# joomanzi/cleisthenes

Hardware: AMD Instinct MI355X
Metric: RBC shard GB/s (RS encode+decode + Merkle verify) per GPU & node, N=128 (higher is better)
Workload: dtype u8

## Files before the change

cleisthenes_amd/csrc/capi.cpp:

```cpp
#include <dlfcn.h>
#include <hip/hip_runtime_api.h>
#include <limits.h>
#include <rccl/rccl.h>
#include <stdio.h>
#include <string.h>

#include <stdlib.h>

#include <algorithm>
#include <functional>
#include <memory>
#include <mutex>
#include <thread>
#include <unordered_map>
#include <vector>

#include "../../include/rbc_gpu.h"
#include "../../include/rbc_protocol.h"
#include "gf_host.h"
#include "kernels.h"
#include "wire_session.h"

namespace {

constexpr size_t kAlign = 64;
inline size_t round_up(size_t x, size_t a) { return (x + a - 1) / a * a; }

int tree_width(int n) {
    int w = 1;
    while (w < n) w <<= 1;
    return w;
}
int tree_depth(int n) {
    int w = tree_width(n), d = 0;
    while ((1 << d) < w) ++d;
    return d;
}

#define RBC_HIP(expr)                                  \
    do {                                               \
        hipError_t e_ = (expr);                        \
        if (e_ != hipSuccess) return RBC_ERR_DEVICE;   \
    } while (0)

struct DevBuf {
    void *p = nullptr;
    size_t cap = 0;
    bool pinned = false;
    hipError_t ensure(size_t bytes) {
        if (bytes <= cap && p) return hipSuccess;
        release();
        size_t want = std::max(bytes, (size_t)256);
        hipError_t e = pinned ? hipHostMalloc(&p, want, hipHostMallocDefault) : hipMalloc(&p, want);
        if (e != hipSuccess) { p = nullptr; cap = 0; return e; }
        cap = want;
        return hipSuccess;
    }
    void release() {
        if (p) {
            if (pinned) (void)hipHostFree(p);
            else (void)hipFree(p);
        }
        p = nullptr;
        cap = 0;
    }
    template <class T> T *as() const { return reinterpret_cast<T *>(p); }
};

struct Ws {
    DevBuf used, regen, dmat, nmiss, flags, list, counter, rcount, cls, vleaves, vlist;
    DevBuf vroot[2], need_full;
    DevBuf rxcnt;
    int rx_par = 0;
    bool rxcnt_init = false, v_clean[2] = {true, true};
    int rx_vslot = 0;
    bool rx_vreuse = false;
    bool fork = true;
    int rx_count = 0;
    const uint8_t *rx_shards = nullptr;
    hipStream_t aux = nullptr;
    hipEvent_t ev_fork = nullptr, ev_join = nullptr, ev_hashed = nullptr, ev_rel = nullptr;
    bool init() {
        return hipEventCreateWithFlags(&ev_fork, hipEventDisableTiming) == hipSuccess &&
               hipEventCreateWithFlags(&ev_join, hipEventDisableTiming) == hipSuccess &&
               hipEventCreateWithFlags(&ev_hashed, hipEventDisableTiming) == hipSuccess &&
               hipEventCreateWithFlags(&ev_rel, hipEventDisableTiming) == hipSuccess;
    }
    void release() {
        for (DevBuf *b : {&used, &regen, &dmat, &nmiss, &flags, &list, &counter, &rcount, &cls, &vleaves, &vlist,
                          &vroot[0], &vroot[1], &need_full, &rxcnt})
            b->release();
        if (aux) (void)hipStreamDestroy(aux);
        if (ev_fork) (void)hipEventDestroy(ev_fork);
        if (ev_join) (void)hipEventDestroy(ev_join);
        if (ev_hashed) (void)hipEventDestroy(ev_hashed);
        if (ev_rel) (void)hipEventDestroy(ev_rel);
        aux = nullptr;
        ev_fork = ev_join = ev_hashed = ev_rel = nullptr;
    }
};

struct Slot {
    DevBuf d_values, d_shards, d_leaves, d_roots, d_branches, d_valid, d_status, d_digests, d_lens, d_slens, d_idx,
        d_offs, d_present, d_pack, d_parity;
    DevBuf h_in{nullptr, 0, true}, h_out{nullptr, 0, true};
    Ws ws;
    hipStream_t stream = nullptr;
    hipEvent_t done = nullptr;
    hipEvent_t kdone = nullptr;
    uint64_t ticket = 0;
    bool busy = false;
    std::function<int()> finish;
    std::function<int(hipStream_t)> d2h;
    int d2h_rc = 0;
    void release() {
        for (DevBuf *b : {&d_values, &d_shards, &d_leaves, &d_roots, &d_branches, &d_valid, &d_status, &d_digests,
                          &d_lens, &d_slens, &d_idx, &d_offs, &d_present, &d_pack, &d_parity, &h_in, &h_out})
            b->release();
        ws.release();
        if (stream) (void)hipStreamDestroy(stream);
        if (done) (void)hipEventDestroy(done);
        if (kdone) (void)hipEventDestroy(kdone);
        stream = nullptr;
        done = nullptr;
        kdone = nullptr;
    }
};

#ifndef RBC_HOST_SLOTS
#define RBC_HOST_SLOTS 4
#endif
constexpr int kHostSlots = RBC_HOST_SLOTS;

}

struct rbc_ctx {
    int n = 0, f = 0, k = 0, p = 0, depth = 0, width = 0, device = 0;
    bool fft = false;
    bool fft_generic = false;
    bool fft_wide = false;
    bool fft_small = false;
    int fft_lane = 0;
    int tx_prio = 0, rx_prio = 0;
    int gemv_prio_ = -1, reencode_prio_ = -1;
    int recheck = RBC_RECHECK_REUSE;
    int wire_codec = RBC_WIRE_CODEC_JSON;
    int gemv_prio() const { return gemv_prio_ < 0 ? tx_prio : gemv_prio_; }
    int reencode_prio() const { return reencode_prio_ < 0 ? tx_prio : reencode_prio_; }
    std::vector<uint8_t> h_M;
    uint8_t *d_M = nullptr;
    std::mutex mu;
    hipStream_t stream = nullptr;
    Ws ws;
    DevBuf d_values, d_shards, d_valid, d_status;
    DevBuf h_stage{nullptr, 0, true};
    uint64_t next_ticket = 1;
    std::vector<std::unique_ptr<Slot>> slots;
    std::unordered_map<uint64_t, int> retired;
    ncclComm_t comm = nullptr;
    int nranks = 1, rank = 0;
    DevBuf d_pack;
};

struct rbc_rs {
    rbc_ctx *ctx = nullptr;
};

namespace {

int ctx_create_kn(int n, int k, int device, rbc_ctx **out) {
    if (!out) return RBC_ERR_INVALID_ARG;
    *out = nullptr;
    if (k <= 0 || n - k < 0) return RBC_ERR_INV_SHARD_NUM;
    if (n > 256) return RBC_ERR_MAX_SHARD_NUM;
    int ndev = 0;
    if (hipGetDeviceCount(&ndev) != hipSuccess || device < 0 || device >= ndev) return RBC_ERR_DEVICE;
    rbc_ctx *c = new rbc_ctx();
    c->n = n;
    c->k = k;
    c->p = n - k;
    c->f = (n - k) / 2;
// ... 183 lines not shown
    return stage_merkle_build(c, st, count, leaves, roots, branches);
}

static bool shared_path_verify(const rbc_ctx *c, const uint32_t *shard_lens, uint32_t uniform_shard_len) {
    const uint32_t blocks_per_row = shard_lens ? 0u : (uniform_shard_len + 9 + 63) / 64;
    return (shard_lens || 16u * (uint32_t)c->depth >= blocks_per_row) && c->depth >= 1;
}

void *ws_buffer(rbc_ctx *c, Ws *wsp, DevBuf Ws::*buf, size_t bytes) {
    std::unique_lock<std::mutex> lk(c->mu, std::defer_lock);
    if (!wsp) lk.lock();
    Ws &w = wsp ? *wsp : c->ws;
    DevBuf &b = w.*buf;
    return b.ensure(bytes) == hipSuccess ? b.p : nullptr;
}

struct EchoVerify {
    uint32_t *counter = nullptr;
    bool zero_counter = true;
    uint8_t *roots_keep = nullptr;
    ShaArgs sha{};
    bool path = false;

    int plan(rbc_ctx *c, hipStream_t st, int count, const Rows &b, const uint8_t *branches, const uint8_t *roots,
             const uint8_t *present, uint8_t *valid, uint8_t *leaves, Ws *wsp) {
        sha = sha_args(c, count, b, leaves, c->rx_prio);
        sha.rows_per_inst = c->n;
        sha.branches = branches;
        sha.br_inst_pitch = (uint64_t)c->n * c->depth * 32;
        sha.roots = roots;
        sha.present = present;
        sha.valid = valid;
        if (present) {
            uint32_t *vl = (uint32_t *)ws_buffer(c, wsp, &Ws::vlist, (size_t)count * c->n * 4 + 64);
            if (!vl) return RBC_ERR_DEVICE;
            uint32_t *vc = counter ? counter : vl + (size_t)count * c->n;
            if (zero_counter) RBC_HIP(hipMemsetAsync(vc, 0, 4, st));
            RBC_HIP(rbc_launch_compact_present(present, c->n, count, valid, vl, vc, st, c->rx_prio,
                                               roots_keep ? roots : nullptr, roots_keep));
            sha.list = vl;
            sha.list_count = vc;
        }
        path = shared_path_verify(c, b.lens, b.uniform_len);
        if (path && !leaves) {
            sha.leaves = (uint8_t *)ws_buffer(c, wsp, &Ws::vleaves, (size_t)count * c->n * 32);
            if (!sha.leaves) return RBC_ERR_DEVICE;
        }
        return RBC_OK;
    }
    int finish(const rbc_ctx *c, hipStream_t st) const {
        if (!path) return RBC_OK;
        PathArgs p{};
        p.count = sha.count;
        p.n = c->n;
        p.width = c->width;
        p.lg_width = c->depth;
        p.depth = c->depth;
        p.leaves = sha.leaves;
        p.leaves_inst_pitch = sha.leaves_inst_pitch;
        p.branches = sha.branches;
        p.br_inst_pitch = sha.br_inst_pitch;
        p.roots = sha.roots;
        p.present = sha.present;
        p.valid = sha.valid;
        p.prio = sha.prio;
        RBC_HIP(rbc_launch_merkle_path(p, st));
        return RBC_OK;
    }
};

int stage_verify(rbc_ctx *c, hipStream_t st, int count, const Rows &b, const uint8_t *branches, const uint8_t *roots,
                 const uint8_t *present, uint8_t *valid, uint8_t *leaves, Ws *wsp = nullptr) {
    if (count < 0 || (count > 0 && (!b.rows || !roots || !valid || (c->depth > 0 && !branches))))
        return RBC_ERR_INVALID_ARG;
    if (!b.rows_ok()) return RBC_ERR_INVALID_ARG;
    if (count == 0) return RBC_OK;
    EchoVerify ev;
    int rc = ev.plan(c, st, count, b, branches, roots, present, valid, leaves, wsp);
    if (rc) return rc;
    RBC_HIP(rbc_launch_sha_rows(ev.sha, !ev.path, st));
    return ev.finish(c, st);
}

int ensure_ws(rbc_ctx *c, Ws &w, int count) {
    const size_t nr = (size_t)std::max(c->n - c->k, 1);
    RBC_HIP(w.used.ensure((size_t)count * c->k));
    RBC_HIP(w.regen.ensure((size_t)count * nr));
    RBC_HIP(w.dmat.ensure((size_t)count * nr * c->k));
    RBC_HIP(w.nmiss.ensure((size_t)count * 4));
    RBC_HIP(w.flags.ensure((size_t)count * c->n * 4));
    RBC_HIP(w.list.ensure((size_t)count * nr * 4));
    RBC_HIP(w.counter.ensure(16));
    RBC_HIP(w.rcount.ensure((size_t)count * 4));
    RBC_HIP(w.cls.ensure((size_t)count * round_up(c->n, 4)));
    return RBC_OK;
}

GfArgs decode_gf_args(const rbc_ctx *c, int count, const Rows &b, const PrepArgs &pa) {
    GfArgs g{};
    g.count = count;
    g.K = c->k;
    g.mode = GF_MODE_DECODE;
    g.in = b.rows;
    g.in_inst_pitch = b.inst_pitch(c);
    g.in_row_pitch = b.pitch;
    g.in_inst_bytes = (uint32_t)b.inst_pitch(c);
    g.out = b.rows;
    g.out_inst_pitch = b.inst_pitch(c);
    g.out_row_pitch = b.pitch;
    g.lens = b.lens;
    g.uniform_len = b.uniform_len;
    g.coef = pa.dmat;
    g.coef_inst_stride = pa.dmat_stride;
    g.in_idx = pa.used;
    g.out_idx = pa.regen;
    g.idx_stride = pa.used_stride;
    g.idx_stride2 = pa.regen_stride;
    g.status = pa.status;
    return g;
}

constexpr uint32_t kFusedJoinMinS = 2048;
int stage_regenerate(rbc_ctx *c, Ws &w, hipStream_t st, int count, const Rows &b, const uint8_t *valid,
                     int32_t *status, int compare = 0, uint32_t *zeroed_counter = nullptr,
                     uint8_t *values_out = nullptr, uint32_t value_pitch = 0, bool *joined = nullptr) {
    if (joined) *joined = false;
    int rc = ensure_ws(c, w, count);
    if (rc) return rc;
    uint32_t *counter = zeroed_counter ? zeroed_counter : w.counter.as<uint32_t>();
    if (compare && !zeroed_counter) RBC_HIP(hipMemsetAsync(counter, 0, 16, st));
    const int nr = c->n - c->k;
    PrepArgs pa{};
    pa.count = count;
    pa.n = c->n;
    pa.k = c->k;
    pa.valid = valid;
    pa.valid_stride = (uint32_t)c->n;
    pa.M = c->d_M;
    pa.used = w.used.as<uint8_t>();
    pa.used_stride = (uint32_t)c->k;
    pa.regen = w.regen.as<uint8_t>();
    pa.regen_stride = (uint32_t)std::max(nr, 1);
    pa.dmat = w.dmat.as<uint8_t>();
    pa.dmat_stride = (uint64_t)std::max(nr, 1) * c->k;
    pa.status = status;
    pa.prio = c->rx_prio;
    if (compare) {
        pa.nmiss = w.nmiss.as<int32_t>();
        pa.flags = w.flags.as<uint32_t>();
        pa.list = w.list.as<uint32_t>();
        pa.counter = counter;
    }
    if (c->fft) {
        pa.fft = 1;
        pa.rcount = w.rcount.as<int32_t>();
        pa.cls = w.cls.as<uint8_t>();
        pa.cls_stride = (uint32_t)round_up(c->n, 4);
        pa.gf_exp = c->d_M + c->h_M.size();
        pa.gf_log = pa.gf_exp + 512;
    }
    RBC_HIP(rbc_launch_decode_prepare(pa, st));
    if (c->fft && nr > 0) {
        const int rmax = std::min(c->k, nr);
        GfArgs g = decode_gf_args(c, count, b, pa);
        g.R = rmax;
        g.rcount = pa.rcount;
        g.prio = c->gemv_prio();
        RBC_HIP(rbc_launch_gf_regen(g, st));
        FftArgs a{};
        a.count = count;
        a.n = c->n;
        a.k = c->k;
        a.mode = GF_MODE_DECODE;
        a.shards = b.rows;
        a.inst_pitch = b.inst_pitch(c);
        a.row_pitch = b.pitch;
        a.lens = b.lens;
        a.uniform_len = b.uniform_len;
        a.status = status;
        a.cls = pa.cls;
        a.cls_stride = pa.cls_stride;
        if (compare) {
            a.flags = pa.flags;
            a.list = pa.list;
            a.counter = pa.counter;
        }
        a.prio = c->reencode_prio();
        a.generic = c->fft_generic;
        a.lane = c->fft_lane;
        if (values_out && joined && !c->fft_generic && !b.lens && b.uniform_len >= kFusedJoinMinS &&
            value_pitch >= (uint64_t)c->k * b.uniform_len &&
            value_pitch - (uint64_t)c->k * b.uniform_len <= std::min<uint64_t>(256, b.pitch)) {
            a.join = values_out;
            a.join_pitch = value_pitch;
            *joined = true;
        }
        RBC_HIP(rbc_launch_rs_fft(a, st));
    } else if (nr > 0) {
        GfArgs g = decode_gf_args(c, count, b, pa);
        g.tiles = (int)((b.pitch + 4095) / 4096);
        g.R = nr;
        g.rc = rbc_gf_pick_rc(nr, kGfRcMax);
        if (compare) {
            g.nmiss = pa.nmiss;
            g.flags = pa.flags;
            g.list = pa.list;
            g.counter = pa.counter;
            g.n = c->n;
        }
        g.prio = c->reencode_prio();
        RBC_HIP(rbc_launch_gf_rows(g, st));
    }
    return RBC_OK;
}

struct JoinBack {
    Ws &w;
    hipStream_t st;
    bool armed = false;
    bool record = true;
    ~JoinBack() {
        if (!armed) return;
        if (record) (void)hipEventRecord(w.ev_join, w.aux);
        (void)hipStreamWaitEvent(st, w.ev_join, 0);
    }
};

int launch_join(rbc_ctx *c, hipStream_t js, int count, const Rows &b, uint8_t *values_out, uint32_t value_pitch,
                const int32_t *status) {
    JoinArgs j{};
    j.count = count;
    j.k = c->k;
// ... 56 lines not shown
        ds = w.aux;
    }
    RBC_HIP(rbc_launch_merkle(m, true, st));
    if (digests)
        RBC_HIP(rbc_launch_digest(leaves, (uint64_t)c->n * 32, c->k, status, digests, count, ds, c->rx_prio));
    return RBC_OK;
}

Rows rx_rows(const rbc_rx_batch *b) { return {b->shards, b->shard_pitch, b->shard_lens, b->uniform_shard_len}; }

int check_rx_batch(rbc_ctx *c, const rbc_rx_batch *b) {
    if (b->count < 0) return RBC_ERR_INVALID_ARG;
    if (b->count == 0) return RBC_OK;
    if (!b->shards || !b->roots || !b->valid || !b->leaves || !b->status || (c->depth > 0 && !b->branches))
        return RBC_ERR_INVALID_ARG;
    return rx_rows(b).decode_ok(c, b->values_out, b->value_pitch) ? RBC_OK : RBC_ERR_INVALID_ARG;
}

bool rx_alias(const rbc_rx_batch *a, const rbc_rx_batch *b) {
    auto same = [](const void *x, const void *y) { return x && x == y; };
    return same(a->shards, b->shards) || same(a->leaves, b->leaves) || same(a->status, b->status) ||
           same(a->valid, b->valid) || same(a->values_out, b->values_out) || same(a->digests, b->digests);
}

int stage_receive_step(rbc_ctx *c, hipStream_t st, const rbc_rx_batch *cur, const rbc_rx_batch *prev,
                       const rbc_rx_marks *marks) {
    Ws &w = c->ws;
    int rc;
    if (cur && (rc = check_rx_batch(c, cur))) return rc;
    if (prev && (rc = check_rx_batch(c, prev))) return rc;
    const bool hc = cur && cur->count > 0, hp = prev && prev->count > 0;
    if (hp != (w.rx_count > 0) || (hp && (prev->count != w.rx_count || prev->shards != w.rx_shards)))
        return RBC_ERR_INVALID_ARG;
    if (hc && hp && rx_alias(cur, prev)) return RBC_ERR_INVALID_ARG;
    if (!hc && !hp) return RBC_OK;
    if (!aux_stream(w)) return RBC_ERR_DEVICE;
    const int nr = c->n - c->k;
    EchoVerify ev;
    ShaArgs r{};
    ev.sha.prio = c->rx_prio;
    RBC_HIP(w.rxcnt.ensure(64));
    if (!w.rxcnt_init) {
        RBC_HIP(hipMemsetAsync(w.rxcnt.p, 0, 64, st));
        w.rxcnt_init = true;
        w.v_clean[0] = w.v_clean[1] = true;
    }
    const int par = w.rx_par;
    uint32_t *cnt = w.rxcnt.as<uint32_t>();
    uint32_t *v_cnt = cnt + 4 * par, *v_next = cnt + 4 * (par ^ 1), *r_cnt = cnt + 8 + 4 * par,
             *r_prev = cnt + 8 + 4 * (par ^ 1);
    const bool reuse = c->recheck == RBC_RECHECK_REUSE && c->depth >= 1;
    const int cur_vslot = w.rx_vslot ^ (hp ? 1 : 0);
    bool roots_kept = false;
    if (hc && reuse) RBC_HIP(w.vroot[cur_vslot].ensure((size_t)cur->count * 32));
    const bool hv = hc && !cur->verified;
    if (hv) {
        ev.counter = v_cnt;
        ev.zero_counter = !w.v_clean[par];
        ev.roots_keep = reuse ? w.vroot[cur_vslot].as<uint8_t>() : nullptr;
        rc = ev.plan(c, st, cur->count, rx_rows(cur), cur->branches, cur->roots, cur->present, cur->valid, cur->leaves,
                     &w);
        if (rc) return rc;
        if (cur->present) {
            w.v_clean[par] = false;
            roots_kept = reuse;
        }
    }
    if (hp && nr > 0) {
        r = sha_args(c, prev->count, rx_rows(prev), prev->leaves, c->rx_prio);
        r.rows_per_inst = nr;
        r.status = prev->status;
        r.list = w.list.as<uint32_t>();
        r.list_count = r_prev;
    }
    if (hc && reuse && !roots_kept)
        RBC_HIP(hipMemcpyAsync(w.vroot[cur_vslot].p, cur->roots, (size_t)cur->count * 32, hipMemcpyDeviceToDevice, st));
    if (marks && marks->hash_begin) RBC_HIP(hipEventRecord((hipEvent_t)marks->hash_begin, st));
    RBC_HIP(rbc_launch_sha_rx(ev.sha, r, hv && !ev.path, st, reinterpret_cast<uint4 *>(r_cnt),
                              reinterpret_cast<uint4 *>(v_next)));
    w.v_clean[par ^ 1] = true;
    if (marks && marks->rows_hashed) RBC_HIP(hipEventRecord((hipEvent_t)marks->rows_hashed, st));
    if ((rc = ev.finish(c, st))) return rc;
    if (marks && marks->hashed) RBC_HIP(hipEventRecord((hipEvent_t)marks->hashed, st));
    JoinBack pj{w, st, false, false};
    if (hp) {
        if (prev->digests) {
            RBC_HIP(hipEventRecord(w.ev_hashed, st));
            RBC_HIP(hipStreamWaitEvent(w.aux, w.ev_hashed, 0));
            RBC_HIP(rbc_launch_digest(prev->leaves, (uint64_t)c->n * 32, c->k, prev->status, prev->digests,
                                      prev->count, w.aux, c->rx_prio));
        }
        RBC_HIP(hipEventRecord(w.ev_join, w.aux));
        pj.armed = true;
        MerkleArgs m = merkle_check_args(c, prev->count, prev->leaves, prev->roots, prev->status);
        if (reuse && w.rx_vreuse) {
            RBC_HIP(w.need_full.ensure((size_t)prev->count));
            RecheckArgs ra{};
            ra.count = prev->count;
            ra.n = c->n;
            ra.width = c->width;
            ra.depth = c->depth;
            ra.leaves = prev->leaves;
            ra.leaves_inst_pitch = (uint64_t)c->n * 32;
            ra.branches = prev->branches;
            ra.br_inst_pitch = (uint64_t)c->n * c->depth * 32;
            ra.valid = prev->valid;
            ra.flags = w.flags.as<uint32_t>();
            ra.vroots = w.vroot[w.rx_vslot].as<uint8_t>();
            ra.expect_roots = prev->roots;
            ra.status = prev->status;
            ra.need_full = w.need_full.as<uint8_t>();
            ra.prio = c->rx_prio;
            RBC_HIP(rbc_launch_recheck(ra, st));
            m.only = ra.need_full;
        }
        RBC_HIP(rbc_launch_merkle(m, true, st));
        if (marks && marks->prev_released) {
            RBC_HIP(hipEventRecord(w.ev_rel, st));
            RBC_HIP(hipStreamWaitEvent(w.aux, w.ev_rel, 0));
            RBC_HIP(hipEventRecord((hipEvent_t)marks->prev_released, w.aux));
        }
    }
    w.rx_count = 0;
    if (hc) {
        if (marks && marks->decode_begin) RBC_HIP(hipEventRecord((hipEvent_t)marks->decode_begin, st));
        bool joined = false;
        rc = stage_regenerate(c, w, st, cur->count, rx_rows(cur), cur->valid, cur->status, 1, r_cnt, cur->values_out,
                              cur->value_pitch, &joined);
        if (rc) return rc;
        if (marks && marks->decoded) RBC_HIP(hipEventRecord((hipEvent_t)marks->decoded, st));
        if (cur->values_out && !joined) {
            RBC_HIP(hipEventRecord(w.ev_fork, st));
            RBC_HIP(hipStreamWaitEvent(w.aux, w.ev_fork, 0));
            rc = launch_join(c, w.aux, cur->count, rx_rows(cur), cur->values_out, cur->value_pitch, cur->status);
            if (rc) return rc;
        }
        w.rx_count = cur->count;
        w.rx_shards = cur->shards;
        w.rx_vslot = cur_vslot;
        w.rx_vreuse = reuse;
    }
    w.rx_par ^= 1;
    return RBC_OK;
}

int check_shards(const size_t *lens, int n, bool nilok, size_t *size_out) {
    size_t size = 0;
    for (int i = 0; i < n; ++i)
        if (lens[i]) { size = lens[i]; break; }
    if (size == 0) return RBC_ERR_SHARD_NO_DATA;
    for (int i = 0; i < n; ++i)
        if (lens[i] != size && (lens[i] != 0 || !nilok)) return RBC_ERR_SHARD_SIZE;
    *size_out = size;
    return RBC_OK;
}

int host_reconstruct(rbc_ctx *c, uint8_t *const *shards, size_t *lens, int n_shards, bool data_only) {
    if (!shards || !lens) return RBC_ERR_INVALID_ARG;
    if (n_shards != c->n) return RBC_ERR_TOO_FEW_SHARDS;
    size_t S = 0;
    int rc = check_shards(lens, n_shards, true, &S);
    if (rc) return rc;
    int present = 0;
    for (int i = 0; i < c->n; ++i) {
        if (lens[i] && !shards[i]) return RBC_ERR_INVALID_ARG;
        present += lens[i] != 0;
    }
    if (present == c->n) return RBC_OK;
    if (present < c->k) return RBC_ERR_TOO_FEW_SHARDS;
    if (S > 0x7fffffffULL / (size_t)c->n) return RBC_ERR_INVALID_ARG;
    const size_t pitch = round_up(S, kAlign);
    std::lock_guard<std::mutex> lk(c->mu);
    RBC_HIP(hipSetDevice(c->device));
    RBC_HIP(c->d_shards.ensure((size_t)c->n * pitch));
    RBC_HIP(c->d_valid.ensure((size_t)c->n));
    RBC_HIP(c->d_status.ensure(sizeof(int32_t)));
    RBC_HIP(c->h_stage.ensure((size_t)c->n * pitch + c->n));
    uint8_t *stage = c->h_stage.as<uint8_t>();
    memset(stage, 0, (size_t)c->n * pitch + c->n);
    for (int i = 0; i < c->n; ++i) {
        if (lens[i]) memcpy(stage + (size_t)i * pitch, shards[i], S);
        stage[(size_t)c->n * pitch + i] = lens[i] ? 1 : 0;
    }
    hipStream_t st = host_stream(c);
    if (!st) return RBC_ERR_DEVICE;
    RBC_HIP(hipMemcpyAsync(c->d_shards.p, stage, (size_t)c->n * pitch, hipMemcpyHostToDevice, st));
    RBC_HIP(hipMemcpyAsync(c->d_valid.p, stage + (size_t)c->n * pitch, c->n, hipMemcpyHostToDevice, st));
    rc = stage_regenerate(c, c->ws, st, 1, {c->d_shards.as<uint8_t>(), (uint32_t)pitch, nullptr, (uint32_t)S},
                          c->d_valid.as<uint8_t>(), c->d_status.as<int32_t>());
    if (rc) return rc;
    RBC_HIP(hipMemcpyAsync(stage, c->d_shards.p, (size_t)c->n * pitch, hipMemcpyDeviceToHost, st));
    int32_t status = 0;
    RBC_HIP(hipMemcpyAsync(&status, c->d_status.p, sizeof status, hipMemcpyDeviceToHost, st));
    RBC_HIP(hipStreamSynchronize(st));
    if (status) return status;
    const int last = data_only ? c->k : c->n;
    for (int i = 0; i < last; ++i) {
        if (lens[i]) continue;
        if (!shards[i]) return RBC_ERR_INVALID_ARG;
        memcpy(shards[i], stage + (size_t)i * pitch, S);
        lens[i] = S;
    }
    return RBC_OK;
}

}

extern "C" {

const char *rbc_strerror(int s) {
    switch (s) {
// ... 1731 lines not shown
```

cleisthenes_amd/csrc/device_common.h:

```cpp
#pragma once
#include <hip/hip_runtime.h>
#include <stdint.h>

#define RBC_DEV __device__ __forceinline__

RBC_DEV void set_wave_prio(int p) {
    if (p == 1) __builtin_amdgcn_s_setprio(1);
    else if (p == 2) __builtin_amdgcn_s_setprio(2);
    else if (p >= 3) __builtin_amdgcn_s_setprio(3);
}

namespace rbcdev {

RBC_DEV uint32_t rotr(uint32_t x, uint32_t n) { return __builtin_amdgcn_alignbit(x, x, n); }
RBC_DEV uint32_t xor3(uint32_t a, uint32_t b, uint32_t c) {
    return __builtin_amdgcn_bitop3_b32(a, b, c, 0x96);
}
RBC_DEV uint32_t bswap32(uint32_t x) { return __builtin_amdgcn_perm(0u, x, 0x00010203u); }
RBC_DEV uint32_t perm(uint32_t hi, uint32_t lo, uint32_t sel) { return __builtin_amdgcn_perm(hi, lo, sel); }

__constant__ static const uint32_t kSHA_K[64] = {
    0x428a2f98, 0x71374491, 0xb5c0fbcf, 0xe9b5dba5, 0x3956c25b, 0x59f111f1, 0x923f82a4, 0xab1c5ed5,
    0xd807aa98, 0x12835b01, 0x243185be, 0x550c7dc3, 0x72be5d74, 0x80deb1fe, 0x9bdc06a7, 0xc19bf174,
    0xe49b69c1, 0xefbe4786, 0x0fc19dc6, 0x240ca1cc, 0x2de92c6f, 0x4a7484aa, 0x5cb0a9dc, 0x76f988da,
// ... 230 lines not shown
#pragma unroll
    for (int r = 0; r < 2; ++r)
#pragma unroll
        for (int t = 0; t < 8; ++t) out[r][t] = s[r].h[t];
}

RBC_DEV void sha256_node64(const uint32_t (&l)[8], const uint32_t (&r)[8], uint32_t (&out)[8]) {
    Sha256State s;
    sha256_init(s);
    uint32_t w[16];
#pragma unroll
    for (int t = 0; t < 8; ++t) { w[t] = l[t]; w[8 + t] = r[t]; }
    sha256_compress(s, w);
#pragma unroll
    for (int t = 0; t < 16; ++t) w[t] = 0;
    w[0] = 0x80000000u;
    w[15] = 512u;
    sha256_compress(s, w);
#pragma unroll
    for (int t = 0; t < 8; ++t) out[t] = s.h[t];
}

RBC_DEV void sha256_node32(const uint32_t (&l)[8], uint32_t (&out)[8]) {
    Sha256State s;
    sha256_init(s);
    uint32_t w[16];
#pragma unroll
    for (int t = 0; t < 8; ++t) w[t] = l[t];
    w[8] = 0x80000000u;
#pragma unroll
    for (int t = 9; t < 15; ++t) w[t] = 0;
    w[15] = 256u;
    sha256_compress(s, w);
#pragma unroll
    for (int t = 0; t < 8; ++t) out[t] = s.h[t];
}

RBC_DEV void sha256_empty(uint32_t (&out)[8]) {
    out[0] = 0xe3b0c442u; out[1] = 0x98fc1c14u; out[2] = 0x9afbf4c8u; out[3] = 0x996fb924u;
    out[4] = 0x27ae41e4u; out[5] = 0x649b934cu; out[6] = 0xa495991bu; out[7] = 0x7852b855u;
}

RBC_DEV void store_digest(uint8_t *dst, const uint32_t (&h)[8]) {
    uint4 *q = reinterpret_cast<uint4 *>(dst);
    q[0] = make_uint4(bswap32(h[0]), bswap32(h[1]), bswap32(h[2]), bswap32(h[3]));
    q[1] = make_uint4(bswap32(h[4]), bswap32(h[5]), bswap32(h[6]), bswap32(h[7]));
}
RBC_DEV void load_digest(const uint8_t *src, uint32_t (&h)[8]) {
    const uint4 *q = reinterpret_cast<const uint4 *>(src);
    const uint4 a = q[0], b = q[1];
    h[0] = bswap32(a.x); h[1] = bswap32(a.y); h[2] = bswap32(a.z); h[3] = bswap32(a.w);
    h[4] = bswap32(b.x); h[5] = bswap32(b.y); h[6] = bswap32(b.z); h[7] = bswap32(b.w);
}

RBC_DEV uint32_t gf_xtime(uint32_t v) { return ((v << 1) ^ ((v & 0x80u) ? 0x1du : 0u)) & 0xffu; }

RBC_DEV void gf_tables(uint32_t c, uint4 &t01, uint32_t &t2) {
    uint32_t m[8];
    m[0] = c & 0xffu;
#pragma unroll
    for (int i = 1; i < 8; ++i) m[i] = gf_xtime(m[i - 1]);
    const uint32_t t0lo = (m[0] << 8) | (m[1] << 16) | ((m[0] ^ m[1]) << 24);
    const uint32_t t0hi = m[2] | ((m[2] ^ m[0]) << 8) | ((m[2] ^ m[1]) << 16) | ((m[2] ^ m[1] ^ m[0]) << 24);
    const uint32_t t1lo = (m[3] << 8) | (m[4] << 16) | ((m[3] ^ m[4]) << 24);
    const uint32_t t1hi = m[5] | ((m[5] ^ m[3]) << 8) | ((m[5] ^ m[4]) << 16) | ((m[5] ^ m[4] ^ m[3]) << 24);
    t01 = make_uint4(t0lo, t0hi, t1lo, t1hi);
    t2 = (m[6] << 8) | (m[7] << 16) | ((m[6] ^ m[7]) << 24);
}

struct GfSel {
    uint32_t s0, s1, s2;
};
RBC_DEV GfSel gf_sel(uint32_t x) {
    GfSel s;
    s.s0 = x & 0x07070707u;
    s.s1 = (x >> 3) & 0x07070707u;
    s.s2 = (x >> 6) & 0x03030303u;
    return s;
}
RBC_DEV uint32_t gf_mul4(const uint4 &t01, uint32_t t2, const GfSel &s) {
    return xor3(perm(t01.y, t01.x, s.s0), perm(t01.w, t01.z, s.s1), perm(t2, t2, s.s2));
}

}
```

cleisthenes_amd/csrc/gf_regen.hip:

```cpp
#include <algorithm>

#include "buffer_io.h"
#include "kernels.h"

using namespace rbcdev;

template <int W>
struct GfVec {
    uint32_t v[W];
};
template <int I, int MAX, class F>
__device__ __forceinline__ void dispatch_rows(int rows, F &&f) {
    if constexpr (I <= MAX) {
        if (rows == I) f(IntC<I>{});
        else dispatch_rows<I + 1, MAX>(rows, f);
    }
}

template <int W, int RC, int JC, int NT, int WPE>
__global__ __launch_bounds__(64 * NT) __attribute__((amdgpu_waves_per_eu(WPE))) void gf_regen_kernel(GfArgs a) {
    static_assert(JC % 4 == 0, "two input pairs per trip");
    static_assert(W >= 1 && W <= 4, "1 to 4 words per lane");
    set_wave_prio(a.prio);
    extern __shared__ __attribute__((aligned(16))) unsigned char smem[];
    const int wave = (int)uniform(threadIdx.x >> 6), lane = (int)(threadIdx.x & 63);
    const int groups = (a.tiles + NT - 1) / NT;
    const int inst = (int)blockIdx.x / groups;
    const int tile = ((int)blockIdx.x - inst * groups) * NT + wave;
    if (inst >= a.count) return;
    if (a.status && a.status[inst] != 0) return;
    const int m = min(a.rcount[inst], a.R);
    if (m <= 0) return;
    const uint32_t pitch = a.out_row_pitch;
    const bool live = tile < a.tiles && (uint32_t)tile * (256u * W) < pitch;
    const uint32_t my_off = (uint32_t)tile * (256u * W) + 4u * W * (uint32_t)lane;
    const uint32_t ld_off = min(my_off, pitch - 4u * W);
    const uint32_t S = inst_len(a.lens, a.uniform_len, inst);
    const int K = a.K;
    const int KP = (K + 3) & ~3;
    constexpr uint32_t T01_B = 16u * RC * JC, T2_B = 8u * RC * (JC / 2), BUF_B = T01_B + T2_B;
    uint32_t *s_off = reinterpret_cast<uint32_t *>(smem + 2 * BUF_B);
    const uint8_t *in_inst = a.in + (size_t)inst * a.in_inst_pitch;
    uint8_t *out_inst = a.out + (size_t)inst * a.out_inst_pitch;
    const rsrc_t rin = make_rsrc(in_inst, a.in_inst_bytes);
    const rsrc_t rout = make_rsrc(out_inst, (uint32_t)a.out_inst_pitch);
    const uint8_t *idx = a.in_idx + (size_t)inst * a.idx_stride;
    for (int t = (int)threadIdx.x; t < KP + 8; t += 64 * NT)
        s_off[t] = (t < K ? (uint32_t)idx[t] : 0u) * a.in_row_pitch;
    __syncthreads();
    const uint8_t *coef = a.coef + (size_t)inst * a.coef_inst_stride;
    const uint8_t *oidx = a.out_idx + (size_t)inst * a.idx_stride2;

    auto load_row = [&](int j) -> GfVec<W> {
        const uint32_t so = uniform(s_off[j]);
        GfVec<W> x;
        if constexpr (W == 4) {
            auto v = __builtin_amdgcn_raw_buffer_load_b128(rin, (int)ld_off, (int)so, 0);
            x.v[0] = v[0]; x.v[1] = v[1]; x.v[2] = v[2]; x.v[3] = v[3];
        } else if constexpr (W == 3) {
            auto v = __builtin_amdgcn_raw_buffer_load_b96(rin, (int)ld_off, (int)so, 0);
            x.v[0] = v[0]; x.v[1] = v[1]; x.v[2] = v[2];
        } else if constexpr (W == 2) {
            auto v = __builtin_amdgcn_raw_buffer_load_b64(rin, (int)ld_off, (int)so, 0);
            x.v[0] = v[0]; x.v[1] = v[1];
        } else {
            x.v[0] = __builtin_amdgcn_raw_buffer_load_b32(rin, (int)ld_off, (int)so, 0);
        }
        return x;
    };

    auto pass = [&](auto rgc, int r0) {
        constexpr int RG = decltype(rgc)::value;
        int tid = (int)threadIdx.x;
        asm volatile("" : "+v"(tid));
        uint32_t acc[RG][W];
#pragma unroll
        for (int r = 0; r < RG; ++r)
#pragma unroll
            for (int w = 0; w < W; ++w) acc[r][w] = 0;
        auto build = [&](int j0, int buf) {
            uint4 *t01s = reinterpret_cast<uint4 *>(smem + buf * BUF_B);
            uint32_t *t2s = reinterpret_cast<uint32_t *>(smem + buf * BUF_B + T01_B);
            for (int e = tid; e < RG * JC; e += 64 * NT) {
                const int jl = e / RG, r = e - jl * RG, j = j0 + jl;
                const uint32_t cf = j < K ? coef[(size_t)(r0 + r) * K + j] : 0u;
                uint4 t01;
                uint32_t t2;
                gf_tables(cf, t01, t2);
                t01s[jl * RC + r] = t01;
                t2s[((jl >> 1) * RC + r) * 2 + (jl & 1)] = t2;
            }
        };
        auto mac_pair = [&](int buf, int jl, const GfVec<W> &xa, const GfVec<W> &xb) {
            GfSel sa[W], sb[W];
#pragma unroll
            for (int w = 0; w < W; ++w) {
                sa[w] = gf_sel(xa.v[w]);
                sb[w] = gf_sel(xb.v[w]);
            }
            uint32_t o01 = (uint32_t)buf * BUF_B + (uint32_t)jl * (16u * RC);
            uint32_t o2 = (uint32_t)buf * BUF_B + T01_B + (uint32_t)(jl >> 1) * (8u * RC);
            asm volatile("" : "+v"(o01), "+v"(o2));
            const unsigned char *p01 = smem + o01;
            const unsigned char *p2 = smem + o2;
#pragma unroll
            for (int r = 0; r < RG; ++r) {
                const uint4 ta = *reinterpret_cast<const uint4 *>(p01 + 16 * r);
                const uint4 tb = *reinterpret_cast<const uint4 *>(p01 + 16 * (RC + r));
                const uint2 t2 = *reinterpret_cast<const uint2 *>(p2 + 8 * r);
#pragma unroll
                for (int w = 0; w < W; ++w)
                    acc[r][w] = xor3(acc[r][w], gf_mul4(ta, t2.x, sa[w]), gf_mul4(tb, t2.y, sb[w]));
            }
        };
        GfVec<W> a0{}, a1{}, b0{}, b1{};
        if (live) {
            a0 = load_row(0);
            a1 = load_row(1);
        }
        for (int j = 0; j < KP; j += 4) {
            const int jl = j % JC, buf = (j / JC) & 1;
            if (jl == 0) {
                build(j, buf);
                __syncthreads();
            }
            if (live) {
                b0 = load_row(j + 2);
                b1 = load_row(j + 3);
                mac_pair(buf, jl, a0, a1);
                a0 = load_row(j + 4);
                a1 = load_row(j + 5);
                mac_pair(buf, jl + 2, b0, b1);
            }
        }
        if (!live) return;
        const int nvalid = (int)S - (int)my_off;
        if (my_off < pitch) {
#pragma unroll
            for (int r = 0; r < RG; ++r) {
                const uint32_t so = uniform((uint32_t)oidx[r0 + r] * pitch);
                uint32_t v[W];
#pragma unroll
                for (int w = 0; w < W; ++w) v[w] = acc[r][w] & keep_bytes(nvalid - 4 * w);
                if constexpr (W == 4) {
                    __builtin_amdgcn_raw_buffer_store_b128(u32x4{v[0], v[1], v[2], v[3]}, rout, (int)my_off, (int)so, 0);
                } else if constexpr (W == 3) {
                    if (my_off + 12u <= pitch) {
                        __builtin_amdgcn_raw_buffer_store_b96(u32x3{v[0], v[1], v[2]}, rout, (int)my_off, (int)so, 0);
                    } else {
#pragma unroll
                        for (int w = 0; w < 3; ++w)
                            if (my_off + 4u * w < pitch)
                                __builtin_amdgcn_raw_buffer_store_b32(v[w], rout, (int)(my_off + 4u * w), (int)so, 0);
                    }
                } else if constexpr (W == 2) {
                    __builtin_amdgcn_raw_buffer_store_b64(u32x2{v[0], v[1]}, rout, (int)my_off, (int)so, 0);
                } else {
                    __builtin_amdgcn_raw_buffer_store_b32(v[0], rout, (int)my_off, (int)so, 0);
                }
            }
        }
    };
    static_assert(RC <= 48, "up to 48 rows a pass");
    for (int r0 = 0; r0 < m; r0 += RC) {
        const int rows = min(RC, m - r0);
        dispatch_rows<1, RC>(rows, [&](auto rgc) { pass(rgc, r0); });
        __syncthreads();
    }
}

hipError_t rbc_launch_gf_regen(const GfArgs &a, hipStream_t st) {
    if (a.count <= 0 || a.R <= 0) return hipSuccess;
    if (a.mode != GF_MODE_DECODE || !a.rcount || a.nmiss || a.copy || a.K < 1 || a.K > 256 || a.out_row_pitch % 4u)
        return hipErrorInvalidValue;
    const RbcRegenForm form = rbc_gf_regen_form(a.lens != nullptr, a.uniform_len, a.out_row_pitch);
    const int W = form.W;
    GfArgs b = a;
    b.wpt = W;
    b.tiles = (int)((a.out_row_pitch + 256u * W - 1) / (256u * W));
    constexpr int JC = 16;
    const int KP = (a.K + 3) & ~3;
    auto go = [&](auto kern) {
        const int RC = form.RC, NT = form.NT;
        const uint64_t blocks = (uint64_t)b.count * ((b.tiles + NT - 1) / NT);
        if (blocks > 0x7fffffffull) return hipErrorInvalidValue;
        const size_t lds = 2 * (size_t)24 * RC * JC + 4 * (size_t)(KP + 8);
        hipLaunchKernelGGL(kern, dim3((unsigned)blocks), dim3(64 * NT), lds, st, b);
        return hipGetLastError();
    };
    if (W == 1)
        return go(gf_regen_kernel<1, kRegenRowsShort, JC, kRegenTilesShort, 4>);
    return go(gf_regen_kernel<2, kRegenRowsLong, JC, kRegenTilesLong, 4>);
}
```

Before: 530.8.

## Move previous-batch recheck and Merkle verify onto aux stream with double-buffered flags

The previous batch's recheck and full Merkle verification now run on the auxiliary stream, so they can overlap with the current batch's decode on the main stream. To avoid a hazard where the current decode-prepare overwrites the flags and need_full buffers the recheck still reads, these buffers are double-buffered and indexed by pipeline parity. This adds an extra event wait and per-slot buffers, and it depends on the JoinBack join to order later work after the aux-stream verification.

```diff
diff --git a/cleisthenes_amd/csrc/capi.cpp b/cleisthenes_amd/csrc/capi.cpp
--- a/cleisthenes_amd/csrc/capi.cpp
+++ b/cleisthenes_amd/csrc/capi.cpp
@@ -68,8 +68,9 @@
 };
 
 struct Ws {
-    DevBuf used, regen, dmat, nmiss, flags, list, counter, rcount, cls, vleaves, vlist;
-    DevBuf vroot[2], need_full;
+    DevBuf used, regen, dmat, nmiss, list, counter, rcount, cls, vleaves, vlist;
+    DevBuf flags[2];
+    DevBuf vroot[2], need_full[2];
     DevBuf rxcnt;
     int rx_par = 0;
     bool rxcnt_init = false, v_clean[2] = {true, true};
@@ -79,24 +80,22 @@
     int rx_count = 0;
     const uint8_t *rx_shards = nullptr;
     hipStream_t aux = nullptr;
-    hipEvent_t ev_fork = nullptr, ev_join = nullptr, ev_hashed = nullptr, ev_rel = nullptr;
+    hipEvent_t ev_fork = nullptr, ev_join = nullptr, ev_hashed = nullptr;
     bool init() {
         return hipEventCreateWithFlags(&ev_fork, hipEventDisableTiming) == hipSuccess &&
                hipEventCreateWithFlags(&ev_join, hipEventDisableTiming) == hipSuccess &&
-               hipEventCreateWithFlags(&ev_hashed, hipEventDisableTiming) == hipSuccess &&
-               hipEventCreateWithFlags(&ev_rel, hipEventDisableTiming) == hipSuccess;
+               hipEventCreateWithFlags(&ev_hashed, hipEventDisableTiming) == hipSuccess;
     }
     void release() {
-        for (DevBuf *b : {&used, &regen, &dmat, &nmiss, &flags, &list, &counter, &rcount, &cls, &vleaves, &vlist,
-                          &vroot[0], &vroot[1], &need_full, &rxcnt})
+        for (DevBuf *b : {&used, &regen, &dmat, &nmiss, &flags[0], &flags[1], &list, &counter, &rcount, &cls, &vleaves,
+                          &vlist, &vroot[0], &vroot[1], &need_full[0], &need_full[1], &rxcnt})
             b->release();
         if (aux) (void)hipStreamDestroy(aux);
         if (ev_fork) (void)hipEventDestroy(ev_fork);
         if (ev_join) (void)hipEventDestroy(ev_join);
         if (ev_hashed) (void)hipEventDestroy(ev_hashed);
-        if (ev_rel) (void)hipEventDestroy(ev_rel);
         aux = nullptr;
-        ev_fork = ev_join = ev_hashed = ev_rel = nullptr;
+        ev_fork = ev_join = ev_hashed = nullptr;
     }
 };
 
@@ -446,13 +445,13 @@
     return ev.finish(c, st);
 }
 
-int ensure_ws(rbc_ctx *c, Ws &w, int count) {
+int ensure_ws(rbc_ctx *c, Ws &w, int count, int fslot) {
     const size_t nr = (size_t)std::max(c->n - c->k, 1);
     RBC_HIP(w.used.ensure((size_t)count * c->k));
     RBC_HIP(w.regen.ensure((size_t)count * nr));
     RBC_HIP(w.dmat.ensure((size_t)count * nr * c->k));
     RBC_HIP(w.nmiss.ensure((size_t)count * 4));
-    RBC_HIP(w.flags.ensure((size_t)count * c->n * 4));
+    RBC_HIP(w.flags[fslot].ensure((size_t)count * c->n * 4));
     RBC_HIP(w.list.ensure((size_t)count * nr * 4));
     RBC_HIP(w.counter.ensure(16));
     RBC_HIP(w.rcount.ensure((size_t)count * 4));
@@ -487,9 +486,9 @@
 constexpr uint32_t kFusedJoinMinS = 2048;
 int stage_regenerate(rbc_ctx *c, Ws &w, hipStream_t st, int count, const Rows &b, const uint8_t *valid,
                      int32_t *status, int compare = 0, uint32_t *zeroed_counter = nullptr,
-                     uint8_t *values_out = nullptr, uint32_t value_pitch = 0, bool *joined = nullptr) {
+                     uint8_t *values_out = nullptr, uint32_t value_pitch = 0, bool *joined = nullptr, int fslot = 0) {
     if (joined) *joined = false;
-    int rc = ensure_ws(c, w, count);
+    int rc = ensure_ws(c, w, count, fslot);
     if (rc) return rc;
     uint32_t *counter = zeroed_counter ? zeroed_counter : w.counter.as<uint32_t>();
     if (compare && !zeroed_counter) RBC_HIP(hipMemsetAsync(counter, 0, 16, st));
@@ -511,7 +510,7 @@
     pa.prio = c->rx_prio;
     if (compare) {
         pa.nmiss = w.nmiss.as<int32_t>();
-        pa.flags = w.flags.as<uint32_t>();
+        pa.flags = w.flags[fslot].as<uint32_t>();
         pa.list = w.list.as<uint32_t>();
         pa.counter = counter;
     }
@@ -734,19 +733,18 @@
     if (marks && marks->rows_hashed) RBC_HIP(hipEventRecord((hipEvent_t)marks->rows_hashed, st));
     if ((rc = ev.finish(c, st))) return rc;
     if (marks && marks->hashed) RBC_HIP(hipEventRecord((hipEvent_t)marks->hashed, st));
-    JoinBack pj{w, st, false, false};
+    JoinBack pj{w, st};
     if (hp) {
-        if (prev->digests) {
-            RBC_HIP(hipEventRecord(w.ev_hashed, st));
-            RBC_HIP(hipStreamWaitEvent(w.aux, w.ev_hashed, 0));
+        RBC_HIP(hipEventRecord(w.ev_hashed, st));
+        RBC_HIP(hipStreamWaitEvent(w.aux, w.ev_hashed, 0));
+        pj.armed = true;
+        if (prev->digests)
             RBC_HIP(rbc_launch_digest(prev->leaves, (uint64_t)c->n * 32, c->k, prev->status, prev->digests,
                                       prev->count, w.aux, c->rx_prio));
-        }
-        RBC_HIP(hipEventRecord(w.ev_join, w.aux));
-        pj.armed = true;
+        const int pslot = par ^ 1;
         MerkleArgs m = merkle_check_args(c, prev->count, prev->leaves, prev->roots, prev->status);
         if (reuse && w.rx_vreuse) {
-            RBC_HIP(w.need_full.ensure((size_t)prev->count));
+            RBC_HIP(w.need_full[pslot].ensure((size_t)prev->count));
             RecheckArgs ra{};
             ra.count = prev->count;
             ra.n = c->n;
@@ -757,28 +755,26 @@
             ra.branches = prev->branches;
             ra.br_inst_pitch = (uint64_t)c->n * c->depth * 32;
             ra.valid = prev->valid;
-            ra.flags = w.flags.as<uint32_t>();
+            ra.flags = w.flags[pslot].as<uint32_t>();
             ra.vroots = w.vroot[w.rx_vslot].as<uint8_t>();
             ra.expect_roots = prev->roots;
             ra.status = prev->status;
-            ra.need_full = w.need_full.as<uint8_t>();
+            ra.need_full = w.need_full[pslot].as<uint8_t>();
             ra.prio = c->rx_prio;
-            RBC_HIP(rbc_launch_recheck(ra, st));
+            RBC_HIP(rbc_launch_recheck(ra, w.aux));
             m.only = ra.need_full;
         }
-        RBC_HIP(rbc_launch_merkle(m, true, st));
-        if (marks && marks->prev_released) {
-            RBC_HIP(hipEventRecord(w.ev_rel, st));
-            RBC_HIP(hipStreamWaitEvent(w.aux, w.ev_rel, 0));
-            RBC_HIP(hipEventRecord((hipEvent_t)marks->prev_released, w.aux));
-        }
+        RBC_HIP(rbc_launch_merkle(m, true, w.aux));
+        RBC_HIP(hipEventRecord(w.ev_join, w.aux));
+        pj.record = false;
+        if (marks && marks->prev_released) RBC_HIP(hipEventRecord((hipEvent_t)marks->prev_released, w.aux));
     }
     w.rx_count = 0;
     if (hc) {
         if (marks && marks->decode_begin) RBC_HIP(hipEventRecord((hipEvent_t)marks->decode_begin, st));
         bool joined = false;
         rc = stage_regenerate(c, w, st, cur->count, rx_rows(cur), cur->valid, cur->status, 1, r_cnt, cur->values_out,
-                              cur->value_pitch, &joined);
+                              cur->value_pitch, &joined, par);
         if (rc) return rc;
         if (marks && marks->decoded) RBC_HIP(hipEventRecord((hipEvent_t)marks->decoded, st));
         if (cur->values_out && !joined) {
```

New measurement: 532.3 (median of 5 runs). No clear change (+0.3%).

## Process GF(256) decode inputs in triples with packed lookup tables

Applied to the files above, without the earlier changes.

Restructures the Reed-Solomon regen MAC loop to consume three input rows per step instead of two. The third coefficient's tables are folded into the spare perm-table slots of the first two, so each output row needs four 2-perm MACs per triple. LDS reads are software-pipelined with a configurable read-ahead depth and fenced with sched barriers. This cuts perm/xor work and LDS traffic per input byte, but it costs extra registers, a third in-flight row load, and changes the chunk size and padding granularity to multiples of six.

```diff
diff --git a/cleisthenes_amd/csrc/device_common.h b/cleisthenes_amd/csrc/device_common.h
--- a/cleisthenes_amd/csrc/device_common.h
+++ b/cleisthenes_amd/csrc/device_common.h
@@ -336,4 +336,36 @@
     return xor3(perm(t01.y, t01.x, s.s0), perm(t01.w, t01.z, s.s1), perm(t2, t2, s.s2));
 }
 
-}
+RBC_DEV void gf_tables3(uint32_t ca, uint32_t cb, uint32_t cc, uint4 (&t)[4]) {
+    uint4 tc;
+    uint32_t t2a, t2b, t2c;
+    gf_tables(ca, t[0], t2a);
+    gf_tables(cb, t[2], t2b);
+    gf_tables(cc, tc, t2c);
+    t[1] = make_uint4(t2a, t2a ^ perm(0u, t2c, 0x01010101u), tc.x, tc.y);
+    t[3] = make_uint4(t2b, t2b ^ perm(0u, t2c, 0x02020202u), tc.z, tc.w);
+}
+struct GfSelHalf {
+    uint32_t s0, s1, s2, s3;
+};
+RBC_DEV GfSelHalf gf_sel3_first(uint32_t a, uint32_t c) {
+    GfSelHalf s;
+    s.s0 = a & 0x07070707u;
+    s.s1 = (a >> 3) & 0x07070707u;
+    s.s2 = ((a >> 6) & 0x03030303u) | ((c >> 4) & 0x04040404u);
+    s.s3 = c & 0x07070707u;
+    return s;
+}
+RBC_DEV GfSelHalf gf_sel3_second(uint32_t b, uint32_t c) {
+    GfSelHalf s;
+    s.s0 = b & 0x07070707u;
+    s.s1 = (b >> 3) & 0x07070707u;
+    s.s2 = ((b >> 6) & 0x03030303u) | ((c >> 5) & 0x04040404u);
+    s.s3 = (c >> 3) & 0x07070707u;
+    return s;
+}
+RBC_DEV uint32_t gf_mac_pair(uint32_t acc, const uint4 &t, uint32_t sx, uint32_t sy) {
+    return xor3(acc, perm(t.y, t.x, sx), perm(t.w, t.z, sy));
+}
+
+}
diff --git a/cleisthenes_amd/csrc/gf_regen.hip b/cleisthenes_amd/csrc/gf_regen.hip
--- a/cleisthenes_amd/csrc/gf_regen.hip
+++ b/cleisthenes_amd/csrc/gf_regen.hip
@@ -17,9 +17,11 @@
     }
 }
 
+constexpr int kRegenReadsAhead = 3;
+
 template <int W, int RC, int JC, int NT, int WPE>
 __global__ __launch_bounds__(64 * NT) __attribute__((amdgpu_waves_per_eu(WPE))) void gf_regen_kernel(GfArgs a) {
-    static_assert(JC % 4 == 0, "two input pairs per trip");
+    static_assert(JC % 6 == 0, "two input triples per trip");
     static_assert(W >= 1 && W <= 4, "1 to 4 words per lane");
     set_wave_prio(a.prio);
     extern __shared__ __attribute__((aligned(16))) unsigned char smem[];
@@ -37,8 +39,8 @@
     const uint32_t ld_off = min(my_off, pitch - 4u * W);
     const uint32_t S = inst_len(a.lens, a.uniform_len, inst);
     const int K = a.K;
-    const int KP = (K + 3) & ~3;
-    constexpr uint32_t T01_B = 16u * RC * JC, T2_B = 8u * RC * (JC / 2), BUF_B = T01_B + T2_B;
+    const int KP = (K + 5) / 6 * 6;
+    constexpr uint32_t BUF_B = 64u * RC * (JC / 3);
     uint32_t *s_off = reinterpret_cast<uint32_t *>(smem + 2 * BUF_B);
     const uint8_t *in_inst = a.in + (size_t)inst * a.in_inst_pitch;
     uint8_t *out_inst = a.out + (size_t)inst * a.out_inst_pitch;
@@ -79,58 +81,71 @@
 #pragma unroll
             for (int w = 0; w < W; ++w) acc[r][w] = 0;
         auto build = [&](int j0, int buf) {
-            uint4 *t01s = reinterpret_cast<uint4 *>(smem + buf * BUF_B);
-            uint32_t *t2s = reinterpret_cast<uint32_t *>(smem + buf * BUF_B + T01_B);
-            for (int e = tid; e < RG * JC; e += 64 * NT) {
-                const int jl = e / RG, r = e - jl * RG, j = j0 + jl;
-                const uint32_t cf = j < K ? coef[(size_t)(r0 + r) * K + j] : 0u;
-                uint4 t01;
-                uint32_t t2;
-                gf_tables(cf, t01, t2);
-                t01s[jl * RC + r] = t01;
-                t2s[((jl >> 1) * RC + r) * 2 + (jl & 1)] = t2;
+            uint4 *ts = reinterpret_cast<uint4 *>(smem + buf * BUF_B);
+            for (int e = tid; e < RG * (JC / 3); e += 64 * NT) {
+                const int tl = e / RG, r = e - tl * RG, j = j0 + 3 * tl;
+                const uint8_t *cr = coef + (size_t)(r0 + r) * K;
+                const uint32_t la = cr[min(j, K - 1)], lb = cr[min(j + 1, K - 1)], lc = cr[min(j + 2, K - 1)];
+                uint4 t[4];
+                gf_tables3(j < K ? la : 0u, j + 1 < K ? lb : 0u, j + 2 < K ? lc : 0u, t);
+                uint4 *d = ts + tl * (4 * RC) + r;
+#pragma unroll
+                for (int q = 0; q < 4; ++q) d[q * RC] = t[q];
             }
         };
-        auto mac_pair = [&](int buf, int jl, const GfVec<W> &xa, const GfVec<W> &xb) {
-            GfSel sa[W], sb[W];
-#pragma unroll
-            for (int w = 0; w < W; ++w) {
-                sa[w] = gf_sel(xa.v[w]);
-                sb[w] = gf_sel(xb.v[w]);
-            }
-            uint32_t o01 = (uint32_t)buf * BUF_B + (uint32_t)jl * (16u * RC);
-            uint32_t o2 = (uint32_t)buf * BUF_B + T01_B + (uint32_t)(jl >> 1) * (8u * RC);
-            asm volatile("" : "+v"(o01), "+v"(o2));
-            const unsigned char *p01 = smem + o01;
-            const unsigned char *p2 = smem + o2;
-#pragma unroll
-            for (int r = 0; r < RG; ++r) {
-                const uint4 ta = *reinterpret_cast<const uint4 *>(p01 + 16 * r);
-                const uint4 tb = *reinterpret_cast<const uint4 *>(p01 + 16 * (RC + r));
-                const uint2 t2 = *reinterpret_cast<const uint2 *>(p2 + 8 * r);
+        auto mac_triple = [&](int buf, int tl, const GfVec<W> &xa, const GfVec<W> &xb, const GfVec<W> &xc) {
+            constexpr int D = kRegenReadsAhead, NU = 4 * RG;
+            uint32_t o = (uint32_t)buf * BUF_B + (uint32_t)tl * (64u * RC);
+            asm volatile("" : "+v"(o));
+            const unsigned char *p = smem + o;
+            uint4 t[D];
+            auto read = [&](int u) {
+                const int h = u / (2 * RG), r = (u >> 1) % RG, q = u & 1;
+                t[u % D] = *reinterpret_cast<const uint4 *>(p + 16 * ((2 * h + q) * RC + r));
+            };
+            GfSelHalf s[W];
+#pragma unroll
+            for (int w = 0; w < W; ++w) s[w] = gf_sel3_first(xa.v[w], xc.v[w]);
+#pragma unroll
+            for (int u = 0; u < D - 1 && u < NU; ++u) read(u);
+#pragma unroll
+            for (int u = 0; u < NU; ++u) {
+                if (u + D - 1 < NU) read(u + D - 1);
+                if (u == 2 * RG) {
+#pragma unroll
+                    for (int w = 0; w < W; ++w) s[w] = gf_sel3_second(xb.v[w], xc.v[w]);
+                }
+                __builtin_amdgcn_sched_barrier(0);
+                const int r = (u >> 1) % RG;
 #pragma unroll
                 for (int w = 0; w < W; ++w)
-                    acc[r][w] = xor3(acc[r][w], gf_mul4(ta, t2.x, sa[w]), gf_mul4(tb, t2.y, sb[w]));
+                    acc[r][w] = u & 1 ? gf_mac_pair(acc[r][w], t[u % D], s[w].s2, s[w].s3)
+                                      : gf_mac_pair(acc[r][w], t[u % D], s[w].s0, s[w].s1);
+                __builtin_amdgcn_sched_barrier(0);
             }
         };
-        GfVec<W> a0{}, a1{}, b0{}, b1{};
+        GfVec<W> a0{}, a1{}, a2{}, b0{}, b1{}, b2{};
         if (live) {
             a0 = load_row(0);
             a1 = load_row(1);
-        }
-        for (int j = 0; j < KP; j += 4) {
+            a2 = load_row(2);
+        }
+        for (int j = 0; j < KP; j += 6) {
             const int jl = j % JC, buf = (j / JC) & 1;
             if (jl == 0) {
                 build(j, buf);
                 __syncthreads();
             }
             if (live) {
-                b0 = load_row(j + 2);
-                b1 = load_row(j + 3);
-                mac_pair(buf, jl, a0, a1);
-                a0 = load_row(j + 4);
-                a1 = load_row(j + 5);
-                mac_pair(buf, jl + 2, b0, b1);
+                const int tl = jl / 3;
+                b0 = load_row(j + 3);
+                b1 = load_row(j + 4);
+                b2 = load_row(j + 5);
+                mac_triple(buf, tl, a0, a1, a2);
+                a0 = load_row(j + 6);
+                a1 = load_row(j + 7);
+                a2 = load_row(j + 8);
+                mac_triple(buf, tl + 1, b0, b1, b2);
             }
         }
         if (!live) return;
@@ -178,13 +193,13 @@
     GfArgs b = a;
     b.wpt = W;
     b.tiles = (int)((a.out_row_pitch + 256u * W - 1) / (256u * W));
-    constexpr int JC = 16;
-    const int KP = (a.K + 3) & ~3;
+    constexpr int JC = 12;
+    const int KP = (a.K + 5) / 6 * 6;
     auto go = [&](auto kern) {
         const int RC = form.RC, NT = form.NT;
         const uint64_t blocks = (uint64_t)b.count * ((b.tiles + NT - 1) / NT);
         if (blocks > 0x7fffffffull) return hipErrorInvalidValue;
-        const size_t lds = 2 * (size_t)24 * RC * JC + 4 * (size_t)(KP + 8);
+        const size_t lds = 2 * (size_t)64 * RC * (JC / 3) + 4 * (size_t)(KP + 8);
         hipLaunchKernelGGL(kern, dim3((unsigned)blocks), dim3(64 * NT), lds, st, b);
         return hipGetLastError();
     };
```

New measurement: 547.1 before, 546.9 after, median of 2. About the same (-0.0%).
